# PRBonn/semantic_suma

Measured on AMD Instinct MI355X. Metric: scans_per_sec, higher is better.
Workload: dtype f32; 1 GPU; BASELINE configs[1]: synthetic KITTI-like sequence, 64x2048 range images, semantic-weighted ICP (10 GN iterations + stats pass) + surfel fusion, one sequence per GPU, scans resident in HBM, processScan called scan after scan by the native host loop (suma_pipeline_run_scans); timed after 300 untimed scans of the same sequence (5 warm-up + pre-roll to the steady map size: 1016645 surfels at the star; preroll_scans=300, map_surfels_start=1016645, map_surfels_end=2308753, parallelism=single GPU

## Files before the change

include/suma_hip.h:

```cpp
#ifndef SUMA_HIP_H_
#define SUMA_HIP_H_

#include <stdint.h>

#include "suma_types.h"

#ifdef __cplusplus
extern "C" {
#endif

enum {
  SUMA_OK = 0,
  SUMA_ERR_INVALID = -1,
  SUMA_ERR_HIP = -2,
  SUMA_ERR_CAPACITY = -3,
  SUMA_ERR_NOMEM = -4
};

typedef struct suma_ctx suma_ctx;
typedef struct suma_frame suma_frame;
typedef struct suma_pipeline suma_pipeline;

const char* suma_version(void);
const char* suma_last_error(const suma_ctx* ctx);
// ... 51 lines not shown
                             float conf_threshold);
suma_frame* suma_map_frame(suma_ctx* ctx, int which);
int suma_map_update_poses(suma_ctx* ctx, const float* poses16, uint32_t n);
int suma_map_size(suma_ctx* ctx, uint32_t* n);
int suma_map_timestamp(suma_ctx* ctx, uint32_t* t);
int suma_map_download(suma_ctx* ctx, suma_surfel* host, uint32_t cap, uint32_t* n);
int suma_map_export_surfels(suma_ctx* ctx, void** d_ptr, uint32_t* n);
int suma_map_export_data_surfels(suma_ctx* ctx, void** d_ptr, uint32_t* first, uint32_t* n_data);
int suma_map_upload(suma_ctx* ctx, const suma_surfel* host, uint32_t n, uint32_t timestamp);
int suma_map_download_index_map(suma_ctx* ctx, uint32_t* host);
int suma_map_download_radius_conf(suma_ctx* ctx, suma_float4* host);
int suma_map_download_integrated(suma_ctx* ctx, uint8_t* host);
int suma_map_counts(suma_ctx* ctx, uint32_t* n_updated, uint32_t* n_new, uint32_t* n_cached, int32_t origin_ij[2]);
int suma_map_download_poses(suma_ctx* ctx, float* host, uint32_t capacity, uint32_t* n);
int suma_map_cache_stats(suma_ctx* ctx, uint32_t* used, uint32_t* capacity, uint32_t* compactions);
int suma_map_download_cached_tile(suma_ctx* ctx, int32_t i, int32_t j, suma_surfel* host, uint32_t capacity, uint32_t* n);

int suma_pipeline_create(const suma_params* params, int hip_device, suma_pipeline** out);
void suma_pipeline_destroy(suma_pipeline* s);
int suma_pipeline_reset(suma_pipeline* s);
suma_ctx* suma_pipeline_ctx(suma_pipeline* s);
int suma_pipeline_process_scan(suma_pipeline* s, const suma_float4* points, const float* labels, const float* probs,
                               uint32_t n, int32_t fixed_iterations);
int suma_pipeline_process_scan_device(suma_pipeline* s, const suma_float4* d_points, const float* d_labels,
                                      const float* d_probs, uint32_t n, int32_t fixed_iterations);
int suma_pipeline_prefetch_scan(suma_pipeline* s, const suma_float4* points, const float* labels, const float* probs,
                                uint32_t n);
int suma_pipeline_process_prefetched(suma_pipeline* s, int32_t fixed_iterations);
int suma_pipeline_process_scan_async(suma_pipeline* s, const suma_float4* points, const float* labels,
                                     const float* probs, uint32_t n, int32_t fixed_iterations);
// ... 486 lines not shown
```

semantic_suma_amd/core.py:

```python
from __future__ import annotations

import ctypes as C
import os

import numpy as np

from .types import (ACC_WORDS, DRAW_COLORS, DRAW_LIGHTS, DRAW_MATERIAL, DRAW_MAX_LIGHTS, SURFEL_DTYPE, DrawParams,
                    IcpStats, LoopParams, LoopStatus, PosegraphParams, PosegraphStats, SemanticKnnParams,
                    SemanticParams, SumaParams, WORLD_SURFEL_DTYPE, WorldParams, WorldStats, CheckpointInfo,
                    ChangeCounts, ChangeParams, ChangeRule, DeskewParams, EVIDENCE_DTYPE, NovelCounts, NovelFuseParams, NovelParams, NovelStats, LocalizerParams, LocalizerResult, PLACE_MAX_MATCHES, PlaceMatch, PlaceParams, RelocalizeResult)

_HERE = os.path.dirname(os.path.abspath(__file__))
LIB_PATH = os.environ.get("SUMA_HIP_LIB") or os.path.join(_HERE, "libsuma_hip.so")
_LIB = None


class SumaError(RuntimeError):
    """Raised for every negative return code of the C-ABI (the reference throws std::runtime_error)."""


class LoopResult(C.Structure):
    _fields_ = [("gn_pose", C.c_double * 16), ("after_minimize", IcpStats), ("passed", C.c_int32),
                ("pose_old", C.c_float * 16), ("composed", IcpStats), ("JtJ", C.c_double * 36)]

# ... 124 lines not shown
    L.suma_map_render_inactive.argtypes = [vp, vp, f32]
    L.suma_map_render_composed.argtypes = [vp, vp, vp, f32]
    L.suma_map_frame.restype = vp
    L.suma_map_frame.argtypes = [vp, C.c_int]
    L.suma_map_update_poses.argtypes = [vp, vp, u32]
    L.suma_map_size.argtypes = [vp, C.POINTER(u32)]
    L.suma_map_timestamp.argtypes = [vp, C.POINTER(u32)]
    L.suma_map_download.argtypes = [vp, vp, u32, C.POINTER(u32)]
    L.suma_map_upload.argtypes = [vp, vp, u32, u32]
    L.suma_map_download_index_map.argtypes = [vp, vp]
    L.suma_map_download_radius_conf.argtypes = [vp, vp]
    L.suma_map_download_poses.argtypes = [vp, vp, u32, C.POINTER(u32)]
    L.suma_map_download_integrated.argtypes = [vp, vp]
    L.suma_map_counts.argtypes = [vp, C.POINTER(u32), C.POINTER(u32), C.POINTER(u32), vp]
    L.suma_map_cache_stats.argtypes = [vp, C.POINTER(u32), C.POINTER(u32), C.POINTER(u32)]
    L.suma_map_download_cached_tile.argtypes = [vp, C.c_int32, C.c_int32, vp, u32, C.POINTER(u32)]
    L.suma_icp_set_iteration.argtypes = [vp, u32]
    L.suma_pipeline_host_entry_times.argtypes = [vp, vp, C.c_int]
    L.suma_loop_closure_verify.argtypes = [vp, vp, vp, vp, u32, vp, f32, f32, f32, C.POINTER(LoopResult)]
    L.suma_loop_closure_verify_serial.argtypes = [vp, vp, vp, vp, u32, vp, f32, f32, f32, C.POINTER(LoopResult)]
    L.suma_pipeline_create.argtypes = [C.POINTER(SumaParams), C.c_int, pp]
    L.suma_pipeline_destroy.argtypes = [vp]
    L.suma_pipeline_destroy.restype = None
    L.suma_pipeline_ctx.restype = vp
    L.suma_pipeline_ctx.argtypes = [vp]
    L.suma_pipeline_process_scan.argtypes = [vp, vp, vp, vp, u32, i32]
    L.suma_pipeline_process_scan_device.argtypes = [vp, vp, vp, vp, u32, i32]
    L.suma_pipeline_pose.argtypes = [vp, vp]
    L.suma_pipeline_begin_scan.argtypes = [vp, vp, vp, vp, u32]
    L.suma_pipeline_begin_scan_device.argtypes = [vp, vp, vp, vp, u32]
# ... 633 lines not shown
        out = np.zeros((p.data_height, p.data_width, 4), dtype=np.float32)
        self.ctx.check(self.ctx.L.suma_map_download_radius_conf(self.ctx.h, _ptr(out)))
        return out

    def integrated(self):
        p = self.ctx.params
        out = np.zeros((p.data_height, p.data_width), dtype=np.uint8)
        self.ctx.check(self.ctx.L.suma_map_download_integrated(self.ctx.h, _ptr(out)))
        return out

    def cache_stats(self):
        a, b, cc = C.c_uint32(0), C.c_uint32(0), C.c_uint32(0)
        self.ctx.check(self.ctx.L.suma_map_cache_stats(self.ctx.h, C.byref(a), C.byref(b), C.byref(cc)))
        return a.value, b.value, cc.value

    def cached_tile(self, i: int, j: int) -> np.ndarray:
        n = C.c_uint32(0)
        self.ctx.check(self.ctx.L.suma_map_download_cached_tile(self.ctx.h, i, j, None, 0, C.byref(n)))
        out = np.zeros((n.value, 16), dtype=np.float32)
        if n.value:
            self.ctx.check(self.ctx.L.suma_map_download_cached_tile(self.ctx.h, i, j, _ptr(out), n.value, C.byref(n)))
        return out

    def cached_tiles(self):
        n = C.c_uint32(0)
        self.ctx.check(self.ctx.L.suma_map_cached_tiles(self.ctx.h, None, 0, C.byref(n)), "suma_map_cached_tiles")
        ij = np.zeros((n.value, 2), dtype=np.int32)
        if n.value:
            self.ctx.check(self.ctx.L.suma_map_cached_tiles(self.ctx.h, _ptr(ij), n.value, C.byref(n)),
                           "suma_map_cached_tiles")
# ... 1023 lines not shown
```

semantic_suma_amd/csrc/k_icp.hip:

```cpp
#include <cstddef>

#include "suma_internal.h"

#ifdef SUMA_GN_TIMING
__device__ unsigned long long g_gn_timing[256][8];
#define GN_STAMP(k)                                                                            \
  do {                                                                                         \
    if (threadIdx.x == 0 && blockIdx.y == 0 && blockIdx.x < 256) g_gn_timing[blockIdx.x][k] = wall_clock64(); \
  } while (0)
extern "C" int suma_debug_gn_timing(unsigned long long* host ) {
  return (int)hipMemcpyFromSymbol(host, HIP_SYMBOL(g_gn_timing), sizeof(g_gn_timing));
}
#else
#define GN_STAMP(k) ((void)0)
#endif

#define ICP_THREADS 512
#define MAGIC_D 6755399441055744.0
#define MAGIC_BITS 0x4338000000000000ll

struct IcpArgs {
  const float4 *Vd, *Nd, *Sd;
  const float4 *Vm, *Nm, *Sm;
  int32_t W, H, Wm, Hm;
// ... 266 lines not shown
  int pixel;
  double* history;
  uint32_t history_cap;
  int init;
  uint32_t iteration0;
  PoseD T0;
  int emit_pose;
  PoseD pose_base;
  float* pose_block;
  HostResult* host_out;
  uint32_t host_seq;
  int host_full;
  const DevState* ds;
  HostResult* fused_report;
  uint32_t* fused_counter;
};

typedef const IterArgs __attribute__((address_space(4))) * IterArgsK;
__device__ __forceinline__ IterArgsK gn_args_again(uint32_t karg_off) {
  const char __attribute__((address_space(4)))* p =
      (const char __attribute__((address_space(4)))*)__builtin_amdgcn_kernarg_segment_ptr() + karg_off;
  asm volatile("" : "+s"(p));
  return (IterArgsK)p;
}

template <bool PIXEL>
__device__ __forceinline__ void icp_iter_body(const IterArgs& g, const uint32_t karg_off) {
  const IcpArgs& a = g.a;
  const GnState* __restrict__ gin = g.gin + blockIdx.y;
  GnState* __restrict__ gout = g.gout + blockIdx.y;
// ... 160 lines not shown
          const int r = lane & 3;
          t = ((s_E[r] * tk_col[0] + s_E[4 + r] * tk_col[1]) + s_E[8 + r] * tk_col[2]) + s_E[12 + r] * tk_col[3];
          if (blockIdx.x == 0 && hist_slot != 0xffffffffu) g.history[16 * (size_t)hist_slot + lane] = t;
        }
        s_pose[lane] = t;
        if (blockIdx.x == 0) gout->Tk[lane] = t;
      }
    }
    GN_STAMP(4);
    __syncthreads();
#pragma unroll
    for (int i = 0; i < 16; ++i) Tk[i] = s_pose[i];
    done = s_flag[0];
    iteration = s_flag[1];
  } else if (writer && g.init) {
    for (int i = 0; i < 16; ++i) gout->Tk[i] = Tk[i];
    if (g.history != nullptr && blockIdx.y == 0)
      for (int i = 0; i < 16; ++i) g.history[i] = Tk[i];
    gout->last_error = (double)3.402823466e+38f;
    gout->F = gout->F_inlier = 0.0;
    gout->iteration = iteration;
    gout->k = 0;
    gout->n_hist = 1;
    gout->converged = 0;
    gout->done = 0;
    gout->valid = gout->outlier = gout->invalid = 0;
  } else if (blockIdx.x == 0 && threadIdx.x < 64 && !g.init) {
    static_assert(sizeof(GnState) % 8 == 0 && offsetof(GnState, pending) % 8 == 0, "GnState is carried as 8-byte words");
    const unsigned long long* __restrict__ src = reinterpret_cast<const unsigned long long*>(gin);
    unsigned long long* __restrict__ dst = reinterpret_cast<unsigned long long*>(gout);
// ... 319 lines not shown
  g.epsilon = ch.epsilon;
  g.delta_thr = ch.delta;
  g.eval_only = eval_only;
  g.pixel = pixel;
  g.history = ch.with_history ? c->gn_history : nullptr;
  g.history_cap = c->gn_history_cap;
  g.emit_pose = (!pixel && ch.pose_base) ? 1 : 0;
  for (int i = 0; i < 16; ++i) g.pose_base.m[i] = ch.pose_base ? ch.pose_base[i] : 0.0;
  g.pose_block = c->pose_block;
  g.host_out = pixel ? nullptr : ch.report;
  g.host_seq = ch.report_seq;
  g.host_full = ch.report_full;
  g.ds = c->ds;
  g.fused_report = self_closing ? ch.report : nullptr;
  g.fused_counter = &c->ds->reserved0;
  g.init = (n_hyp == 1 && c->gn_launch == 0) ? 1 : 0;
  g.iteration0 = ch.iteration0;
  for (int i = 0; i < 16; ++i) g.T0.m[i] = g.init ? ch.T0s[i] : 0.0;
  c->gn_launch += 1;
  dim3 grid(pixel ? c->icp_blocks : 1, n_hyp);
  if (pixel)
    k_icp_step<<<grid, ICP_THREADS, 0, c->ls>>>(g.pin, g.gin, g.a.Vd, g.a.Nd, g.a.Sd, g);
  else
    k_icp_finish<<<grid, ICP_THREADS, 0, c->ls>>>(g.pin, g.gin, g);
  return hipGetLastError();
}

const GnState* gn_result(suma_ctx* c) { return gn_buf(c, c->gn_launch); }
```

semantic_suma_amd/csrc/k_sync.hip:

```cpp
#include <atomic>
#include <cstddef>
#include <cstdlib>

#include "suma_internal.h"

__global__ void k_signal(uint32_t* word, uint32_t seq) {
  __hip_atomic_store(word, seq, __ATOMIC_RELEASE, __HIP_MEMORY_SCOPE_AGENT);
}

__global__ void k_gate(const uint32_t* word, uint32_t seq, uint32_t* fault) {
  if (threadIdx.x != 0) return;
  for (uint32_t spins = 0; spins < (1u << 24); ++spins) {
    if ((int32_t)(__hip_atomic_load(word, __ATOMIC_ACQUIRE, __HIP_MEMORY_SCOPE_AGENT) - seq) >= 0) return;
    __builtin_amdgcn_s_sleep(16);
  }
  atomicOr(fault, 8u);
  atomicOr(fault + (offsetof(DevState, fault_site) - offsetof(DevState, overflow)) / 4, 0x1u);
}

hipError_t launch_signal(suma_ctx* c, hipStream_t st, uint32_t word, uint32_t seq) {
  k_signal<<<1, 1, 0, st>>>(c->sync_flags + word, seq);
  return hipGetLastError();
}
hipError_t launch_gate(suma_ctx* c, hipStream_t st, uint32_t word, uint32_t seq) {
  k_gate<<<1, 64, 0, st>>>(c->sync_flags + word, seq, &c->ds->overflow);
  return hipGetLastError();
}
static std::atomic<int> g_side_ctxs(0);

int ensure_side_stream(suma_ctx* c) {
  if (c->side_stream || c->side_stream_off) return SUMA_OK;
  const char* ser = getenv("AMD_SERIALIZE_KERNEL");
  const bool serialised = getenv("ROCPROF_COUNTER_COLLECTION") != nullptr || (ser && atoi(ser) != 0);
  if (getenv("SUMA_NO_SIDE_STREAM") || serialised) {
    c->side_stream_off = 1;
    return SUMA_OK;
  }
  HIP_TRY(c, hipStreamCreateWithFlags(&c->side_stream, hipStreamNonBlocking));
  g_side_ctxs.fetch_add(1);
  HIP_TRY(c, hipEventCreateWithFlags(&c->pre_event, hipEventDisableTiming));
  HIP_TRY(c, hipEventCreateWithFlags(&c->order_event, hipEventDisableTiming));
  HIP_TRY(c, c->zbuf_k1.alloc(c->P));
  HIP_TRY(c, hipMemsetAsync(c->zbuf_k1, 0xFF, c->P * 8, c->stream));
  HIP_TRY(c, hipStreamSynchronize(c->stream));
  return SUMA_OK;
}
void side_stream_released(suma_ctx* c) {
  if (c->side_stream) g_side_ctxs.fetch_sub(1);
}

int side_handoff(suma_ctx* c, const suma_frame* frame) {
  static const bool force_events = getenv("SUMA_GATE_EVENTS") != nullptr;
  c->pre_seq += 1;
  if (force_events || g_side_ctxs.load() > 1) {
    HIP_TRY(c, hipEventRecord(c->pre_event, c->side_stream));
    c->gate_by_event = 1;
  } else {
    HIP_TRY(c, launch_signal(c, c->side_stream, 0, c->pre_seq));
    c->gate_by_event = 0;
  }
  c->gate_pending = c->pre_seq;
  c->gate_frame = frame;
  return SUMA_OK;
}

hipError_t flush_gate(suma_ctx* c) {
  if (!c->gate_pending) return hipSuccess;
  const uint32_t seq = c->gate_pending;
  c->gate_pending = 0;
  c->gate_frame = nullptr;
  if (c->gate_by_event) return hipStreamWaitEvent(c->stream, c->pre_event, 0);
  return launch_gate(c, c->stream, 0, seq);
}
```

semantic_suma_amd/csrc/k_update.hip:

```cpp
#include <cstddef>
#include <cstring>

#include "suma_internal.h"

#define ST_AGG 1u
#define ST_INC 2u

__device__ __forceinline__ unsigned long long st_pack(uint32_t epoch, uint32_t flag, uint32_t value) {
  return ((unsigned long long)epoch << 34) | ((unsigned long long)flag << 32) | value;
}

struct Pair {
  uint32_t a, x;
};
__device__ __forceinline__ void lookback_publish(unsigned long long* __restrict__ status,
                                                 unsigned long long* __restrict__ group, uint32_t tile, uint32_t agg,
                                                 uint32_t epoch, uint32_t aggx = 0) {
  __hip_atomic_store(&status[tile], st_pack(epoch, ST_AGG, (aggx << 16) | agg), __ATOMIC_RELAXED, __HIP_MEMORY_SCOPE_AGENT);
  __hip_atomic_fetch_add(&group[tile >> 6], (1ull << 56) | ((unsigned long long)aggx << 32) | (unsigned long long)agg,
                         __ATOMIC_RELAXED, __HIP_MEMORY_SCOPE_AGENT);
}
#define SUMA_SPIN_LIMIT (1u << 26)
#ifndef LB_BATCH
#define LB_BATCH 4
// ... 868 lines not shown
  a.x_arena = xf ? c->cache_arena : nullptr;
  a.x_slots = c->cache_slots;
  a.x_cap = c->cache_cap;
  a.x_slot = xf ? (uint32_t)fused_slot : 0u;
  a.ex_cx = ex ? ex[0] : 0.0f;
  a.ex_cy = ex ? ex[1] : 0.0f;
  a.ex_extent = ex ? ex[2] : 0.0f;
  hipStream_t st = c->ls;
  const uint32_t gridS = stream_grid(c, (uint64_t)c->known_surfels + 2 * c->P);
  a.pose_idx = c->timestamp;
  a.write_pose = 0;
  if (c->k8_fused_frame == f && c->k8_fused_stamp == c->timestamp && c->k8_fused_params == c->params_version) {
    a.write_pose = 1;
  } else {
    ProfScope ps(c, "k8_radius", 48.0 * P);
    k8_radius<<<(P + 255) / 256, 256, 0, st>>>(a.V, a.N, launch_k8_out(c), P, c->ds, c->poses, c->poses_inv, c->timestamp,
                                                a.pose, a.Sem);
  }
  c->k8_fused_frame = nullptr;
  if (!k7_done) {
    ProfScope ps(c, "k7_indexmap", 64.0 * S + 8.0 * P);
    k7_indexmap<<<gridS, 256, 0, st>>>(a);
  }
  {
    ProfScope ps(c, "k9_update_surfels", 128.0 * S + 16.0 * P);
    a.epoch = ++c->epoch;
    a.group = c->tile_group + (size_t)(a.epoch & 1u) * c->group_words;
    a.group_next = c->tile_group + (size_t)((a.epoch + 1u) & 1u) * c->group_words;
    const uint32_t grid = compact_grid(c, (uint64_t)c->known_surfels + 2 * c->P);
    if (xf)
// ... 239 lines not shown
```

semantic_suma_amd/csrc/suma_api.hip:

```cpp
#include <cmath>
#include <cstdio>
#include <cstring>
#include <mutex>
#include <new>
#include <set>

#include <time.h>

#include "suma_internal.h"

static std::mutex g_ctx_mu;
static std::set<const suma_ctx*> g_live_ctx;
static bool ctx_alive(const suma_ctx* c) {
  std::lock_guard<std::mutex> lk(g_ctx_mu);
  return g_live_ctx.count(c) != 0;
}

static thread_local std::string g_create_error;

extern "C" const char* suma_version(void) { return "suma-hip 0.1 (gfx950)"; }
extern "C" const char* suma_last_error(const suma_ctx* ctx) { return ctx ? ctx->err.c_str() : g_create_error.c_str(); }
int fail_without_ctx(int code, const std::string& msg) {
  g_create_error = msg;
  return code;
// ... 638 lines not shown
  const suma_frame* cur = c->icp_current;
  const bool k8_wanted = cur->width == c->p.data_width && cur->height == c->p.data_height &&
                         !(c->k8_fused_frame == cur && c->k8_fused_version == cur->version &&
                           c->k8_fused_stamp == c->timestamp && c->k8_fused_params == c->params_version);
  HostResult* rec = &c->h_rec[1];
  c->rec_seq += 1;
  ch.report = rec;
  ch.report_seq = c->rec_seq;
  ch.report_full = 1;
  ch.fuse_k8 = k8_wanted ? 1 : 0;
  {
    ProfScope ps(c, k8_wanted ? "k6k8_stats_radius" : "k6_icp_step", (96.0 + (k8_wanted ? 81.0 : 0.0)) * (double)cur->width * cur->height);
    CK(launch_icp_iteration(c, ch, 1, 1));
  }
  if (k8_wanted) {
    c->k8_fused_frame = cur;
    c->k8_fused_version = cur->version;
    c->k8_fused_stamp = c->timestamp;
    c->k8_fused_params = c->params_version;
  }
  const uint64_t mark = c->enq_seq;
  int r = wait_host_result(c, rec, c->rec_seq);
  if (r) return r;
  c->done_seq = mark;
  unpack_acc(c, *rec, JtJ, Jtr, acc);
  fill_stats_host(*rec, stats);
  if (stats) stats->iterations = 0;
  return SUMA_OK;
}

// ... 771 lines not shown

static int resolve_stats(suma_pipeline* s, bool need_sync);

extern "C" int suma_pipeline_create(const suma_params* params, int hip_device, suma_pipeline** out) {
  if (!params || !out) return SUMA_ERR_INVALID;
  *out = nullptr;
  suma_ctx* c = nullptr;
  int r = suma_ctx_create(params, hip_device, &c);
  if (r) return r;
  suma_pipeline* s = new (std::nothrow) suma_pipeline();
  if (!s) {
    suma_ctx_destroy(c);
    return SUMA_ERR_NOMEM;
  }
  s->c = c;
  suma_frame** fr[4] = {&s->last_frame, &s->current_frame, &s->current_model, &s->last_model};
  for (int k = 0; k < 4; ++k) {
    bool data = k < 2;
    r = frame_create_raw(c, data ? params->data_width : params->model_width,
                         data ? params->data_height : params->model_height, fr[k]);
    if (r) {
      g_create_error = c->err;
      suma_pipeline_destroy(s);
      return r;
    }
  }
  if (s->h_res.alloc(3) != hipSuccess) {
    g_create_error = "hipHostMalloc failed";
    suma_pipeline_destroy(s);
    return SUMA_ERR_HIP;
  }
  memset(s->h_res, 0, 3 * sizeof(HostResult));
  if (ensure_side_stream(c) != SUMA_OK) {
// ... 4 lines not shown
  mat4_eye(s->current_pose);
  mat4_eye(s->last_pose);
  mat4_eye(s->pose_old);
  mat4_eye(s->pose_new);
  mat4_eye(s->last_increment);
  mat4_eye(s->last_pose_old);
  float p_unstable = 0.1f;
  s->log_unstable = (float)log((double)(p_unstable / (1.0f - p_unstable)));
  *out = s;
  return SUMA_OK;
}
extern "C" void suma_pipeline_destroy(suma_pipeline* s) {
  if (!s) return;
  loop_destroy(s);
  ingest_destroy(s->c);
  if (s->c && s->c->stream) hipStreamSynchronize(s->c->stream);
  suma_frame_destroy(s->last_frame);
  suma_frame_destroy(s->current_frame);
  suma_frame_destroy(s->current_model);
  suma_frame_destroy(s->last_model);
  deskew_destroy(s);
  suma_ctx_destroy(s->c);
  delete s;
}
extern "C" suma_ctx* suma_pipeline_ctx(suma_pipeline* s) { return s ? s->c : nullptr; }
extern "C" int suma_pipeline_pose(const suma_pipeline* s, double pose[16]) {
  if (!s || !pose) return SUMA_ERR_INVALID;
  memcpy(pose, s->current_pose, 16 * sizeof(double));
  return SUMA_OK;
}
extern "C" int suma_pipeline_last_increment(const suma_pipeline* s, double inc[16]) {
  if (!s || !inc) return SUMA_ERR_INVALID;
  memcpy(inc, s->last_increment, 16 * sizeof(double));
// ... 67 lines not shown
  CK(hipMemcpyAsync(c->h_gn, gn_result(c), sizeof(GnState), hipMemcpyDeviceToHost, c->stream));
  CK(hipMemcpyAsync(c->h_ds, c->ds, sizeof(DevState), hipMemcpyDeviceToHost, c->stream));
  for (;;) {
    hipError_t q = hipStreamQuery(c->stream);
    if (q == hipSuccess) break;
    if (q != hipErrorNotReady) CK(q);
  }
  int rs = resolve_stats(s, false);
  if (rs) return rs;
  c->known_surfels = c->h_ds->n_surfels;
  memcpy(T, c->h_gn[0].Tk, 16 * sizeof(double));
  fill_stats(c->h_gn[0], st);
  return check_overflow(c);
}

static int update_pose(suma_pipeline* s, int32_t fixed_iterations) {
  suma_ctx* c = s->c;
  double T0[16], increment[16];
  if (!c->p.initialize_identity)
    memcpy(T0, s->last_increment, sizeof(T0));
  else
    mat4_eye(T0);
  suma_icp_stats mst;
  {
    GnChain ch = pipeline_chain(s, c->new_frame, T0, 1, fixed_iterations, false);
    ch.pose_base = s->pose_new;
    s->res_seq += 1;
    ch.report = &s->h_res[0];
    ch.report_seq = s->res_seq;
    int r0 = enqueue_minimize(c, ch);
    if (r0) return r0;
  }
  c->rendered.valid = false;
  CK(launch_map_render_single(c, nullptr, conf_threshold(s), 1, 1, s->last_model));
  c->new_frame->version++;
  s->last_model->version++;
  double I[16];
  mat4_eye(I);
  GnChain st = gn_chain_ctx(c, I, 1);
  CK(launch_gn_init(c, st));
  const uint32_t slot = s->stats_slot ^ 1u;
  {
    ProfScope ps(c, "k6k8_stats_radius", (96.0 + 81.0) * (double)c->P);
    st.report = &s->h_res[1 + slot];
    st.report_seq = s->res_seq;
    st.fuse_k8 = 1;
    CK(launch_icp_iteration(c, st, 1, 1));
    c->k8_fused_frame = s->current_frame;
    c->k8_fused_version = s->current_frame->version;
    c->k8_fused_stamp = c->timestamp;
    c->k8_fused_params = c->params_version;
  }
  struct timespec tw0, tw1;
  clock_gettime(CLOCK_MONOTONIC, &tw0);
  int r = wait_host_result(c, &s->h_res[0], s->res_seq);
  clock_gettime(CLOCK_MONOTONIC, &tw1);
  c->het.result_wait_s += (double)(tw1.tv_sec - tw0.tv_sec) + 1e-9 * (double)(tw1.tv_nsec - tw0.tv_nsec);
  if (r) return r;
  r = resolve_stats(s, false);
  if (r) return r;
  s->stats_slot = slot;
  *c->h_ds = s->h_res[0].ds;
  c->known_surfels = c->h_ds->n_surfels;
  memcpy(increment, s->h_res[0].Tk, sizeof(increment));
  fill_stats_host(s->h_res[0], &mst);
  r = check_overflow(c);
// ... 31 lines not shown
  memcpy(s->pose_new, np, sizeof(np));
  memcpy(s->last_increment, increment, sizeof(increment));
  return SUMA_OK;
}

int pipeline_begin_scan_impl(suma_pipeline* s, const suma_float4* d_points, const float* d_labels, const float* d_probs,
                             uint32_t n, hipEvent_t upload_done) {
  if (!s || (n > 0 && !d_points)) return SUMA_ERR_INVALID;
  suma_ctx* c = s->c;
  if (s->phase != 0) return fail(c, SUMA_ERR_INVALID, "suma_pipeline_begin_scan: the previous scan has not been closed with suma_pipeline_update_map");
  c->obj_set = false;
  if (s->loop) {
    int ri = loop_integrate(s);
    if (ri) return ri;
  }
  std::swap(s->last_frame, s->current_frame);
  std::swap(s->last_model, s->current_model);
  int r;
  const bool deskew = s->deskew && s->deskew->on;
  if (c->side_stream) {
    if (upload_done) HIP_TRY(c, hipStreamWaitEvent(c->side_stream, upload_done, 0));
    if (deskew && (r = deskew_scan(c, *s->deskew, s->last_increment, c->side_stream, d_points, n, &d_points)) != SUMA_OK) return r;
    c->ls = c->side_stream;
    r = suma_preprocess_device(c, d_points, d_labels, d_probs, n, s->timestamp, s->current_frame);
    c->ls = c->stream;
    if (r) return r;
    r = side_handoff(c, s->current_frame);
    if (r) return r;
  } else {
    if (upload_done) HIP_TRY(c, hipStreamWaitEvent(c->stream, upload_done, 0));
    if (deskew && (r = deskew_scan(c, *s->deskew, s->last_increment, c->stream, d_points, n, &d_points)) != SUMA_OK) return r;
    r = suma_preprocess_device(c, d_points, d_labels, d_probs, n, s->timestamp, s->current_frame);
    if (r) return r;
  }
// ... 1 lines not shown
  mat4_cast_f(s->pose_old, po);
  mat4_cast_f(s->pose_new, pn);
  r = map_render_dedup(c, po, pn, conf_threshold(s), s->last_model);
  if (r) return r;
  s->phase = 1;
  return SUMA_OK;
}

int pipeline_update_pose_impl(suma_pipeline* s, int32_t fixed_iterations) {
  if (!s) return SUMA_ERR_INVALID;
  if (s->phase != 1) return fail(s->c, SUMA_ERR_INVALID, "suma_pipeline_update_pose: call suma_pipeline_begin_scan first");
  if (s->timestamp > 0) {
    int r = update_pose(s, fixed_iterations);
    if (r) return r;
    if (s->loop && (r = loop_odometry_edge(s)) != SUMA_OK) return r;
  }
  s->phase = 2;
  return SUMA_OK;
}

int pipeline_update_map_impl(suma_pipeline* s) {
  if (!s) return SUMA_ERR_INVALID;
  suma_ctx* c = s->c;
  if (s->phase != 2) return fail(c, SUMA_ERR_INVALID, "suma_pipeline_update_map: call suma_pipeline_update_pose first");
  float pc[16];
  mat4_cast_f(s->current_pose, pc);
  int r = suma_map_update(c, pc, s->current_frame);
  if (r) return r;
  r = map_render_dedup(c, pc, pc, conf_threshold(s), s->current_model);
  if (r) return r;
// ... 20 lines not shown
extern "C" int suma_pipeline_begin_scan_device(suma_pipeline* s, const suma_float4* d_points, const float* d_labels,
                                               const float* d_probs, uint32_t n) {
  return pipeline_begin_scan_impl(s, d_points, d_labels, d_probs, n, nullptr);
}
extern "C" int suma_pipeline_update_pose(suma_pipeline* s, int32_t fixed_iterations) {
  return pipeline_update_pose_impl(s, fixed_iterations);
}
extern "C" int suma_pipeline_update_map(suma_pipeline* s) { return pipeline_update_map_impl(s); }

extern "C" int suma_pipeline_reset(suma_pipeline* s) {
  if (!s) return SUMA_ERR_INVALID;
  suma_ctx* c = s->c;
  int r = suma_synchronize(c);
  if (r) return r;
  if (c->gate_pending) c->gate_pending = 0;
  host_synced(c);
  ingest_drain(c);
  r = map_reset_impl(c);
  if (r) return r;
  r = loop_reset(s);
  if (r) return r;
  s->stats_pending = false;
  memset(&s->stats, 0, sizeof(s->stats));
  s->timestamp = 0;
  s->track_loss = 0;
  s->phase = 0;
  mat4_eye(s->current_pose);
  mat4_eye(s->last_pose);
  mat4_eye(s->pose_old);
  mat4_eye(s->pose_new);
// ... 87 lines not shown
                                 min_valid_ratio, max_outlier_ratio, max_increment_difference, out);
}

extern "C" int suma_pipeline_process_scan_device(suma_pipeline* s, const suma_float4* d_points, const float* d_labels,
                                                 const float* d_probs, uint32_t n, int32_t fixed_iterations) {
  return pipeline_process_scan_impl(s, d_points, d_labels, d_probs, n, fixed_iterations, nullptr);
}

extern "C" int suma_pipeline_process_scan(suma_pipeline* s, const suma_float4* points, const float* labels,
                                          const float* probs, uint32_t n, int32_t fixed_iterations) {
  if (!s || (n > 0 && !points)) return SUMA_ERR_INVALID;
  suma_ctx* c = s->c;
  (void)c;
  return pipeline_process_host_scan(s, points, labels, probs, n, fixed_iterations);
}
```

semantic_suma_amd/csrc/suma_internal.h:

```cpp
#ifndef SUMA_INTERNAL_H_
#define SUMA_INTERNAL_H_

#include <hip/hip_runtime.h>
#include <math.h>
#include <stdint.h>

#include <initializer_list>
#include <map>
#include <string>
#include <utility>
#include <vector>

#include "../../include/suma_hip.h"
#include "dev_math.h"

#ifndef SUMA_TILE
#define SUMA_TILE 1024u
#endif
#ifndef SUMA_COMPACT_BLOCKS
#define SUMA_COMPACT_BLOCKS 256u
#endif
#define SUMA_STREAM_BLOCKS 2048u
#define SUMA_EXTRACT_CAPACITY 500000u
#define SUMA_MAX_MODEL_WIDTH 5461u
// ... 84 lines not shown

struct GnChain {
  const suma_frame *current, *model;
  suma_icp_objective obj;
  uint32_t max_iterations;
  double epsilon, delta;
  const double* T0s;
  uint32_t n_hyp;
  uint32_t iteration0, iteration0_rest;
  int with_history;
  HostResult* report;
  uint32_t report_seq;
  int report_full;
  const double* pose_base;
  int fuse_k8;
};

struct MapConsts {
  float pixel_size, log_prior, log_unstable, p_unstable;
  float radconf_angle_thresh, update_angle_thresh;
};

struct suma_frame {
  suma_ctx* ctx;
  uint32_t width, height;
  DevBuf<float4> block;
  float4* map[3];
  uint64_t version;
  uint64_t last_access;
};
// ... 14 lines not shown
  double result_wait_s;
  double call_s;
  uint64_t calls;
  uint32_t copy_threads;
};

struct suma_ctx {
  suma_params p;
  int device;
  hipStream_t stream;
  hipStream_t ls;
  hipStream_t side_stream;
  int side_stream_off;
  DevBuf<uint32_t> sync_flags;
  uint32_t pre_seq;
  uint32_t gate_pending;
  int gate_by_event;
  hipEvent_t pre_event;
  hipEvent_t order_event;
  uint64_t enq_seq, done_seq;
  bool cache_nothing_stale;
  const suma_frame* gate_frame;
  struct Ingest* ingest;
  PinnedBuf<HostResult> h_rec;
  uint32_t rec_seq;
  std::string err;

  proj_t pd, pm;
  MapConsts mc;
  size_t P, Pm;
// ... 99 lines not shown
    float last_pose[16];
    uint64_t map_version, params_version;
  } k7_spec;
  struct {
    bool valid;
    float pose_old[16], pose_new[16], conf_threshold;
    uint64_t map_version, params_version;
    const suma_frame* out;
    uint64_t out_version, old_version, new_version;
  } rendered;
};

struct suma_pipeline {
  suma_ctx* c;
  suma_frame *last_frame, *current_frame, *current_model, *last_model;
  double current_pose[16], last_pose[16], pose_old[16], pose_new[16], last_increment[16];
  double last_pose_old[16];
  uint32_t timestamp;
  int phase;
  float log_unstable;
  suma_icp_stats stats;
  uint32_t track_loss;
  PinnedBuf<HostResult> h_res;
  uint32_t res_seq, stats_seq;
  bool stats_pending;
  uint32_t stats_slot;
  suma_icp_stats stats_mst;
  struct LoopState* loop;
  struct Deskew* deskew;
};
// ... 8 lines not shown
hipStream_t pipeline_input_stream(suma_pipeline* s);
int fail(suma_ctx* c, int code, const std::string& msg);
int fail_without_ctx(int code, const std::string& msg);
int check_overflow(suma_ctx* c);
int semantic_check(suma_ctx* c, const suma_semantic_params* sp);
int semantic_scan_input(suma_pipeline* s, uint32_t n, void* producer_event, hipStream_t* st);
void ingest_destroy(suma_ctx* c);
void ingest_drain(suma_ctx* c);
uint32_t ingest_pending(suma_ctx* c);
int ingest_stage_blocking(suma_ctx* c, const suma_float4* points, const float* labels, const float* probs, uint32_t n,
                          const suma_float4** d_points, const float** d_labels, const float** d_probs, hipEvent_t* uploaded,
                          void** slot);
void ingest_consumed(suma_ctx* c, void* slot, hipStream_t reader);
int ensure_side_stream(suma_ctx* c);
int side_handoff(suma_ctx* c, const suma_frame* frame);
void side_stream_released(suma_ctx* c);
int pipeline_process_host_scan(suma_pipeline* s, const suma_float4* points, const float* labels, const float* probs,
                               uint32_t n, int32_t fixed_iterations);

#define HIP_TRY(ctx, expr)                                                                       \
  do {                                                                                           \
    hipError_t e__ = (expr);                                                                     \
    if (e__ != hipSuccess) {                                                                     \
      (ctx)->err = std::string(#expr) + ": " + hipGetErrorString(e__);                           \
      return SUMA_ERR_HIP;                                                                       \
    }                                                                                            \
  } while (0)

template <class T, bool Pinned>
int grow(suma_ctx* c, DevBuf<T, Pinned>& b, size_t n, std::initializer_list<hipStream_t> drain, size_t alloc = 0) {
// ... 213 lines not shown
```

semantic_suma_amd/csrc/suma_runner.hip:

```cpp
#include <string.h>

#include <atomic>
#include <chrono>
#include <string>
#include <thread>
#include <vector>

#include <hip/hip_runtime.h>

#include "../../include/suma_runner.h"
#include "suma_internal.h"

static double now_s() {
  return std::chrono::duration<double>(std::chrono::steady_clock::now().time_since_epoch()).count();
}
static void set_error(char* dst, size_t cap, const std::string& msg) {
  if (!dst || !cap) return;
  strncpy(dst, msg.c_str(), cap - 1);
  dst[cap - 1] = 0;
}

static void run_one_sequence(suma_pipeline* s, const suma_sequence_job& job, int32_t fixed_iterations,
                             suma_sequence_result* res) {
  memset(res, 0, sizeof(*res));
// ... 24 lines not shown
  suma_pipeline_pose(s, res->end_pose);
  res->track_loss = suma_pipeline_track_loss(s);
  uint32_t n = 0;
  if (suma_map_size(suma_pipeline_ctx(s), &n) == SUMA_OK) res->map_surfels = n;
}

extern "C" int suma_pipeline_run_scans(suma_pipeline* s, const suma_sequence_job* job, int32_t fixed_iterations,
                                       uint32_t* scans_done, double* seconds_per_call) {
  if (!s || !job || (!job->scans && job->n_scans)) return SUMA_ERR_INVALID;
  SUMA_REFUSE_WHILE_DESKEW(s, "suma_pipeline_run_scans");
  int r = SUMA_OK;
  uint32_t k = 0;
  double t_prev = seconds_per_call ? now_s() : 0.0;
  for (; k < job->n_scans && r == SUMA_OK; ++k) {
    const suma_scan_ref& sc = job->scans[k];
    r = job->on_device ? suma_pipeline_process_scan_device(s, sc.points, sc.labels, sc.probs, sc.n, fixed_iterations)
                       : suma_pipeline_process_scan(s, sc.points, sc.labels, sc.probs, sc.n, fixed_iterations);
    if (seconds_per_call) {
      const double t = now_s();
      seconds_per_call[k] = t - t_prev;
      t_prev = t;
    }
  }
  if (scans_done) *scans_done = (r == SUMA_OK) ? k : (k ? k - 1 : 0);
  return r;
}

extern "C" int suma_run_sequences(const suma_params* params, int hip_device, const suma_sequence_job* jobs,
                                  uint32_t n_jobs, uint32_t max_concurrent, int32_t fixed_iterations,
                                  suma_sequence_result* results) {
  if (!params || (!jobs && n_jobs) || (!results && n_jobs)) return SUMA_ERR_INVALID;
  if (n_jobs == 0) return SUMA_OK;
  if (max_concurrent == 0) max_concurrent = 1;
  const uint32_t n_workers = max_concurrent < n_jobs ? max_concurrent : n_jobs;
  std::atomic<uint32_t> next(0);
  auto worker = [&]() {
    suma_pipeline* s = nullptr;
    int rc = (hipSetDevice(hip_device) == hipSuccess) ? suma_pipeline_create(params, hip_device, &s) : SUMA_ERR_HIP;
// ... 127 lines not shown
```

Before: 2912 scans/s.

## Preprocess next scan on side stream during current scan's ICP

```diff
diff --git a/include/suma_hip.h b/include/suma_hip.h
--- a/include/suma_hip.h
+++ b/include/suma_hip.h
@@ -89,6 +89,7 @@
 int suma_map_counts(suma_ctx* ctx, uint32_t* n_updated, uint32_t* n_new, uint32_t* n_cached, int32_t origin_ij[2]);
 int suma_map_download_poses(suma_ctx* ctx, float* host, uint32_t capacity, uint32_t* n);
 int suma_map_cache_stats(suma_ctx* ctx, uint32_t* used, uint32_t* capacity, uint32_t* compactions);
+int suma_debug_launch_counts(const suma_ctx* ctx, uint32_t out[3]);
 int suma_map_download_cached_tile(suma_ctx* ctx, int32_t i, int32_t j, suma_surfel* host, uint32_t capacity, uint32_t* n);
 
 int suma_pipeline_create(const suma_params* params, int hip_device, suma_pipeline** out);
diff --git a/semantic_suma_amd/core.py b/semantic_suma_amd/core.py
--- a/semantic_suma_amd/core.py
+++ b/semantic_suma_amd/core.py
@@ -162,6 +162,7 @@
     L.suma_map_download_integrated.argtypes = [vp, vp]
     L.suma_map_counts.argtypes = [vp, C.POINTER(u32), C.POINTER(u32), C.POINTER(u32), vp]
     L.suma_map_cache_stats.argtypes = [vp, C.POINTER(u32), C.POINTER(u32), C.POINTER(u32)]
+    L.suma_debug_launch_counts.argtypes = [vp, C.POINTER(u32)]
     L.suma_map_download_cached_tile.argtypes = [vp, C.c_int32, C.c_int32, vp, u32, C.POINTER(u32)]
     L.suma_icp_set_iteration.argtypes = [vp, u32]
     L.suma_pipeline_host_entry_times.argtypes = [vp, vp, C.c_int]
@@ -825,6 +826,11 @@
         self.ctx.check(self.ctx.L.suma_map_cache_stats(self.ctx.h, C.byref(a), C.byref(b), C.byref(cc)))
         return a.value, b.value, cc.value
 
+    def launch_counts(self):
+        out = (C.c_uint32 * 3)()
+        self.ctx.check(self.ctx.L.suma_debug_launch_counts(self.ctx.h, out))
+        return out[0], out[1], out[2]
+
     def cached_tile(self, i: int, j: int) -> np.ndarray:
         n = C.c_uint32(0)
         self.ctx.check(self.ctx.L.suma_map_download_cached_tile(self.ctx.h, i, j, None, 0, C.byref(n)))
diff --git a/semantic_suma_amd/csrc/k_icp.hip b/semantic_suma_amd/csrc/k_icp.hip
--- a/semantic_suma_amd/csrc/k_icp.hip
+++ b/semantic_suma_amd/csrc/k_icp.hip
@@ -304,6 +304,8 @@
   const DevState* ds;
   HostResult* fused_report;
   uint32_t* fused_counter;
+  uint32_t* start_word;
+  uint32_t start_seq;
 };
 
 typedef const IterArgs __attribute__((address_space(4))) * IterArgsK;
@@ -494,6 +496,11 @@
     done = s_flag[0];
     iteration = s_flag[1];
   } else if (writer && g.init) {
+    if (PIXEL) {
+      const IterArgsK gk = gn_args_again(karg_off);
+      uint32_t* const sw = gk->start_word;
+      if (sw != nullptr) __hip_atomic_store(sw, gk->start_seq, __ATOMIC_RELAXED, __HIP_MEMORY_SCOPE_AGENT);
+    }
     for (int i = 0; i < 16; ++i) gout->Tk[i] = Tk[i];
     if (g.history != nullptr && blockIdx.y == 0)
       for (int i = 0; i < 16; ++i) g.history[i] = Tk[i];
@@ -843,6 +850,8 @@
   g.ds = c->ds;
   g.fused_report = self_closing ? ch.report : nullptr;
   g.fused_counter = &c->ds->reserved0;
+  g.start_word = (pixel && !eval_only && n_hyp == 1 && c->gn_launch == 0) ? ch.start_word : nullptr;
+  g.start_seq = ch.start_seq;
   g.init = (n_hyp == 1 && c->gn_launch == 0) ? 1 : 0;
   g.iteration0 = ch.iteration0;
   for (int i = 0; i < 16; ++i) g.T0.m[i] = g.init ? ch.T0s[i] : 0.0;
diff --git a/semantic_suma_amd/csrc/k_sync.hip b/semantic_suma_amd/csrc/k_sync.hip
--- a/semantic_suma_amd/csrc/k_sync.hip
+++ b/semantic_suma_amd/csrc/k_sync.hip
@@ -4,8 +4,9 @@
 
 #include "suma_internal.h"
 
-__global__ void k_signal(uint32_t* word, uint32_t seq) {
+__global__ void k_signal(uint32_t* word, uint32_t seq, uint32_t* host_word) {
   __hip_atomic_store(word, seq, __ATOMIC_RELEASE, __HIP_MEMORY_SCOPE_AGENT);
+  if (host_word) __hip_atomic_store(host_word, seq, __ATOMIC_RELEASE, __HIP_MEMORY_SCOPE_SYSTEM);
 }
 
 __global__ void k_gate(const uint32_t* word, uint32_t seq, uint32_t* fault) {
@@ -19,7 +20,7 @@
 }
 
 hipError_t launch_signal(suma_ctx* c, hipStream_t st, uint32_t word, uint32_t seq) {
-  k_signal<<<1, 1, 0, st>>>(c->sync_flags + word, seq);
+  k_signal<<<1, 1, 0, st>>>(c->sync_flags + word, seq, word == 0 ? c->side_done_h.p : nullptr);
   return hipGetLastError();
 }
 hipError_t launch_gate(suma_ctx* c, hipStream_t st, uint32_t word, uint32_t seq) {
@@ -40,6 +41,8 @@
   g_side_ctxs.fetch_add(1);
   HIP_TRY(c, hipEventCreateWithFlags(&c->pre_event, hipEventDisableTiming));
   HIP_TRY(c, hipEventCreateWithFlags(&c->order_event, hipEventDisableTiming));
+  HIP_TRY(c, c->side_done_h.alloc(1));
+  *c->side_done_h = 0;
   HIP_TRY(c, c->zbuf_k1.alloc(c->P));
   HIP_TRY(c, hipMemsetAsync(c->zbuf_k1, 0xFF, c->P * 8, c->stream));
   HIP_TRY(c, hipStreamSynchronize(c->stream));
@@ -49,10 +52,22 @@
   if (c->side_stream) g_side_ctxs.fetch_sub(1);
 }
 
+static bool force_events() {
+  static const bool on = getenv("SUMA_GATE_EVENTS") != nullptr;
+  return on;
+}
+bool side_handoff_in_memory(void) { return !force_events() && g_side_ctxs.load() <= 1; }
+
+int side_handoff_ahead(suma_ctx* c, uint32_t* seq) {
+  c->pre_seq += 1;
+  HIP_TRY(c, launch_signal(c, c->side_stream, 0, c->pre_seq));
+  *seq = c->pre_seq;
+  return SUMA_OK;
+}
+
 int side_handoff(suma_ctx* c, const suma_frame* frame) {
-  static const bool force_events = getenv("SUMA_GATE_EVENTS") != nullptr;
   c->pre_seq += 1;
-  if (force_events || g_side_ctxs.load() > 1) {
+  if (!side_handoff_in_memory()) {
     HIP_TRY(c, hipEventRecord(c->pre_event, c->side_stream));
     c->gate_by_event = 1;
   } else {
@@ -70,5 +85,12 @@
   c->gate_pending = 0;
   c->gate_frame = nullptr;
   if (c->gate_by_event) return hipStreamWaitEvent(c->stream, c->pre_event, 0);
+  if ((int32_t)(c->gate_waited - seq) >= 0) return hipSuccess;
+  if (c->side_done_h) {
+    const bool seen = (int32_t)(__atomic_load_n(c->side_done_h.p, __ATOMIC_ACQUIRE) - seq) >= 0;
+    if (seen) return hipSuccess;
+  }
+  c->gate_waited = seq;
+  c->dbg_ctx_gates += 1;
   return launch_gate(c, c->stream, 0, seq);
 }
diff --git a/semantic_suma_amd/csrc/k_update.hip b/semantic_suma_amd/csrc/k_update.hip
--- a/semantic_suma_amd/csrc/k_update.hip
+++ b/semantic_suma_amd/csrc/k_update.hip
@@ -906,6 +906,7 @@
     a.write_pose = 1;
   } else {
     ProfScope ps(c, "k8_radius", 48.0 * P);
+    c->dbg_k8_launches += 1;
     k8_radius<<<(P + 255) / 256, 256, 0, st>>>(a.V, a.N, launch_k8_out(c), P, c->ds, c->poses, c->poses_inv, c->timestamp,
                                                 a.pose, a.Sem);
   }
diff --git a/semantic_suma_amd/csrc/suma_api.hip b/semantic_suma_amd/csrc/suma_api.hip
--- a/semantic_suma_amd/csrc/suma_api.hip
+++ b/semantic_suma_amd/csrc/suma_api.hip
@@ -676,6 +676,7 @@
     CK(launch_icp_iteration(c, ch, 1, 1));
   }
   if (k8_wanted) {
+    c->dbg_k8_launches += 1;
     c->k8_fused_frame = cur;
     c->k8_fused_version = cur->version;
     c->k8_fused_stamp = c->timestamp;
@@ -1477,9 +1478,9 @@
     return SUMA_ERR_NOMEM;
   }
   s->c = c;
-  suma_frame** fr[4] = {&s->last_frame, &s->current_frame, &s->current_model, &s->last_model};
-  for (int k = 0; k < 4; ++k) {
-    bool data = k < 2;
+  suma_frame** fr[5] = {&s->last_frame, &s->current_frame, &s->ahead_frame, &s->current_model, &s->last_model};
+  for (int k = 0; k < 5; ++k) {
+    bool data = k < 3;
     r = frame_create_raw(c, data ? params->data_width : params->model_width,
                          data ? params->data_height : params->model_height, fr[k]);
     if (r) {
@@ -1514,9 +1515,11 @@
   if (!s) return;
   loop_destroy(s);
   ingest_destroy(s->c);
+  if (s->c && s->c->side_stream) hipStreamSynchronize(s->c->side_stream);
   if (s->c && s->c->stream) hipStreamSynchronize(s->c->stream);
   suma_frame_destroy(s->last_frame);
   suma_frame_destroy(s->current_frame);
+  suma_frame_destroy(s->ahead_frame);
   suma_frame_destroy(s->current_model);
   suma_frame_destroy(s->last_model);
   deskew_destroy(s);
@@ -1614,6 +1617,30 @@
   return check_overflow(c);
 }
 
+static bool lookahead_possible(const suma_pipeline* s) {
+  static const bool off = getenv("SUMA_NO_LOOKAHEAD") != nullptr;
+  const suma_ctx* c = s->c;
+  return !off && s->next_scan && c->side_stream && side_handoff_in_memory() && !s->loop && !(s->deskew && s->deskew->on) &&
+         !(s->next_scan->n > 0 && !s->next_scan->points);
+}
+static int preprocess_ahead(suma_pipeline* s, bool gated) {
+  suma_ctx* c = s->c;
+  const suma_pipeline::AheadScan sc = *s->next_scan;
+  s->ahead.valid = false;
+  if (gated) CK(launch_gate(c, c->side_stream, 1, c->start_seq));
+  c->ls = c->side_stream;
+  int r = suma_preprocess_device(c, sc.points, sc.labels, sc.probs, sc.n, s->timestamp + 1, s->ahead_frame);
+  c->ls = c->stream;
+  if (r) return r;
+  r = side_handoff_ahead(c, &s->ahead.seq);
+  if (r) return r;
+  s->ahead.scan = sc;
+  s->ahead.timestamp = s->timestamp + 1;
+  s->ahead.params_version = c->params_version;
+  s->ahead.valid = true;
+  return SUMA_OK;
+}
+
 static int update_pose(suma_pipeline* s, int32_t fixed_iterations) {
   suma_ctx* c = s->c;
   double T0[16], increment[16];
@@ -1622,9 +1649,15 @@
   else
     mat4_eye(T0);
   suma_icp_stats mst;
+  const bool ahead = lookahead_possible(s);
   {
     GnChain ch = pipeline_chain(s, c->new_frame, T0, 1, fixed_iterations, false);
     ch.pose_base = s->pose_new;
+    if (ahead) {
+      c->start_seq += 1;
+      ch.start_word = c->sync_flags + 1;
+      ch.start_seq = c->start_seq;
+    }
     s->res_seq += 1;
     ch.report = &s->h_res[0];
     ch.report_seq = s->res_seq;
@@ -1645,11 +1678,16 @@
     st.report = &s->h_res[1 + slot];
     st.report_seq = s->res_seq;
     st.fuse_k8 = 1;
+    c->dbg_k8_launches += 1;
     CK(launch_icp_iteration(c, st, 1, 1));
     c->k8_fused_frame = s->current_frame;
     c->k8_fused_version = s->current_frame->version;
     c->k8_fused_stamp = c->timestamp;
     c->k8_fused_params = c->params_version;
+  }
+  if (ahead) {
+    int ra = preprocess_ahead(s, true);
+    if (ra) return ra;
   }
   struct timespec tw0, tw1;
   clock_gettime(CLOCK_MONOTONIC, &tw0);
@@ -1711,10 +1749,33 @@
     int ri = loop_integrate(s);
     if (ri) return ri;
   }
+  const bool deskew = s->deskew && s->deskew->on;
+  const bool made_ahead = s->ahead.valid && !upload_done && !deskew && s->ahead.scan.points == d_points &&
+                          s->ahead.scan.labels == d_labels && s->ahead.scan.probs == d_probs && s->ahead.scan.n == n &&
+                          s->ahead.timestamp == s->timestamp && s->ahead.params_version == c->params_version &&
+                          !c->gate_pending;
+  s->ahead.valid = false;
+  if (made_ahead) {
+    suma_frame* spare = s->last_frame;
+    s->last_frame = s->current_frame;
+    s->current_frame = s->ahead_frame;
+    s->ahead_frame = spare;
+    std::swap(s->last_model, s->current_model);
+    c->gate_pending = s->ahead.seq;
+    c->gate_by_event = 0;
+    c->gate_frame = s->current_frame;
+    c->dbg_frames_ahead += 1;
+    float po[16], pn[16];
+    mat4_cast_f(s->pose_old, po);
+    mat4_cast_f(s->pose_new, pn);
+    int rr = map_render_dedup(c, po, pn, conf_threshold(s), s->last_model);
+    if (rr) return rr;
+    s->phase = 1;
+    return SUMA_OK;
+  }
   std::swap(s->last_frame, s->current_frame);
   std::swap(s->last_model, s->current_model);
   int r;
-  const bool deskew = s->deskew && s->deskew->on;
   if (c->side_stream) {
     if (upload_done) HIP_TRY(c, hipStreamWaitEvent(c->side_stream, upload_done, 0));
     if (deskew && (r = deskew_scan(c, *s->deskew, s->last_increment, c->side_stream, d_points, n, &d_points)) != SUMA_OK) return r;
@@ -1746,6 +1807,11 @@
     int r = update_pose(s, fixed_iterations);
     if (r) return r;
     if (s->loop && (r = loop_odometry_edge(s)) != SUMA_OK) return r;
+  } else if (lookahead_possible(s)) {
+    suma_ctx* c = s->c;
+    int r = preprocess_ahead(s, false);
+    if (r) return r;
+    if (c->gate_pending && !c->gate_by_event) c->gate_pending = s->ahead.seq;
   }
   s->phase = 2;
   return SUMA_OK;
@@ -1796,6 +1862,8 @@
   int r = suma_synchronize(c);
   if (r) return r;
   if (c->gate_pending) c->gate_pending = 0;
+  s->ahead.valid = false;
+  s->next_scan = nullptr;
   host_synced(c);
   ingest_drain(c);
   r = map_reset_impl(c);
@@ -1913,3 +1981,11 @@
   (void)c;
   return pipeline_process_host_scan(s, points, labels, probs, n, fixed_iterations);
 }
+
+extern "C" int suma_debug_launch_counts(const suma_ctx* c, uint32_t out[3]) {
+  if (!c || !out) return SUMA_ERR_INVALID;
+  out[0] = c->dbg_ctx_gates;
+  out[1] = c->dbg_k8_launches;
+  out[2] = c->dbg_frames_ahead;
+  return SUMA_OK;
+}
diff --git a/semantic_suma_amd/csrc/suma_internal.h b/semantic_suma_amd/csrc/suma_internal.h
--- a/semantic_suma_amd/csrc/suma_internal.h
+++ b/semantic_suma_amd/csrc/suma_internal.h
@@ -122,6 +122,8 @@
   int report_full;
   const double* pose_base;
   int fuse_k8;
+  uint32_t* start_word;
+  uint32_t start_seq;
 };
 
 struct MapConsts {
@@ -166,6 +168,11 @@
   int side_stream_off;
   DevBuf<uint32_t> sync_flags;
   uint32_t pre_seq;
+  PinnedBuf<uint32_t> side_done_h;
+  uint32_t gate_waited;
+  uint32_t start_seq;
+  uint32_t dbg_frames_ahead;
+  uint32_t dbg_ctx_gates, dbg_k8_launches;
   uint32_t gate_pending;
   int gate_by_event;
   hipEvent_t pre_event;
@@ -295,6 +302,21 @@
 struct suma_pipeline {
   suma_ctx* c;
   suma_frame *last_frame, *current_frame, *current_model, *last_model;
+  suma_frame* ahead_frame;
+  struct AheadScan {
+    const suma_float4* points;
+    const float *labels, *probs;
+    uint32_t n;
+  };
+  const AheadScan* next_scan;
+  AheadScan next_scan_store;
+  struct {
+    bool valid;
+    AheadScan scan;
+    uint32_t timestamp;
+    uint64_t params_version;
+    uint32_t seq;
+  } ahead;
   double current_pose[16], last_pose[16], pose_old[16], pose_new[16], last_increment[16];
   double last_pose_old[16];
   uint32_t timestamp;
@@ -333,6 +355,8 @@
 void ingest_consumed(suma_ctx* c, void* slot, hipStream_t reader);
 int ensure_side_stream(suma_ctx* c);
 int side_handoff(suma_ctx* c, const suma_frame* frame);
+int side_handoff_ahead(suma_ctx* c, uint32_t* seq);
+bool side_handoff_in_memory(void);
 void side_stream_released(suma_ctx* c);
 int pipeline_process_host_scan(suma_pipeline* s, const suma_float4* points, const float* labels, const float* probs,
                                uint32_t n, int32_t fixed_iterations);
diff --git a/semantic_suma_amd/csrc/suma_runner.hip b/semantic_suma_amd/csrc/suma_runner.hip
--- a/semantic_suma_amd/csrc/suma_runner.hip
+++ b/semantic_suma_amd/csrc/suma_runner.hip
@@ -62,14 +62,21 @@
   double t_prev = seconds_per_call ? now_s() : 0.0;
   for (; k < job->n_scans && r == SUMA_OK; ++k) {
     const suma_scan_ref& sc = job->scans[k];
+    if (job->on_device && k + 1 < job->n_scans) {
+      const suma_scan_ref& nx = job->scans[k + 1];
+      s->next_scan_store = {nx.points, nx.labels, nx.probs, nx.n};
+      s->next_scan = &s->next_scan_store;
+    }
     r = job->on_device ? suma_pipeline_process_scan_device(s, sc.points, sc.labels, sc.probs, sc.n, fixed_iterations)
                        : suma_pipeline_process_scan(s, sc.points, sc.labels, sc.probs, sc.n, fixed_iterations);
+    s->next_scan = nullptr;
     if (seconds_per_call) {
       const double t = now_s();
       seconds_per_call[k] = t - t_prev;
       t_prev = t;
     }
   }
+  s->ahead.valid = false;
   if (scans_done) *scans_done = (r == SUMA_OK) ? k : (k ? k - 1 : 0);
   return r;
 }
```

New measurement: 2872 scans/s. 1.4% lower.
